# thethomasboyer/PhenDiff

Measured on AMD Instinct MI355X. Metric: img2img images/sec (50-step DDIM invert+denoise, 256x256), higher is better.
Workload: dtype bf16; 1 GPU; configs[2]: 256x256 pipeline_conditional_ddim invert->class-swap->denoise, 50+50 DDIM steps, super_small UNet (random init, seed 0), 3k_steps_clipping_rescaling, 32 images/GPU/step sharded over 1 GPU(s), no collectives; batch_per_gpu=32, global_batch=32, inference_steps=50, image_size=256, hipgraph=True, concurrent_trajectories=1

## Files before the change

### phendiff_amd/csrc/conv_igemm.hip

```cpp
#include <type_traits>
#include <utility>
#include <stdio.h>
#include <stdlib.h>
#include "pd_common.h"
#include "pd_stage.h"
#include "pd_conv.h"

namespace pd {

constexpr int CONV_AR8 = 6;
constexpr int CONV_PRO_DEFAULT = 1;
constexpr int CONV_PRO_WPS = 3;
constexpr int CONV_PRO_START = 8;
template <int... I, typename F> __device__ __forceinline__ void pd_static_for_impl(std::integer_sequence<int, I...>, F&& f) { (f(std::integral_constant<int, I>{}), ...); }
template <int N, typename F> __device__ __forceinline__ void pd_static_for(F&& f) { pd_static_for_impl(std::make_integer_sequence<int, N>{}, f); }
constexpr int PRO_OPS = 37;
constexpr int pro_op_cost(int k) {
  if (k >= 36) return 100;
  const int stg = (k % 18) >> 1;
  return (stg == 3 || stg == 4 || stg == 6 || stg == 7) ? 87 : (stg == 0 ? 60 : (stg == 8 ? 106 : 58));
}
constexpr int pro_ops_done(int S, int NS, int PS0, int NIT) {
  if (S < PS0) return 0;
  if (S >= NS - 1) return NIT * PRO_OPS;
  long long tot = 0;
  for (int k = 0; k < PRO_OPS; ++k) tot += pro_op_cost(k);
  tot *= NIT;
  const long long target = (long long)(S - PS0 + 1) * tot / (NS - PS0);
  int done = 0;
  long long dc = 0;
  while (done < NIT * PRO_OPS && dc + pro_op_cost(done % PRO_OPS) <= target) { dc += pro_op_cost(done % PRO_OPS); ++done; }
  return done;
}
__device__ __forceinline__ unsigned pd_lin_block() { return blockIdx.x + gridDim.x * (blockIdx.y + gridDim.y * blockIdx.z); }
template <typename T, int KS, int STRIDE, int TH, int TW, bool DB, bool TAIL, int NCO = 1, bool PLAIN = false, int PRO = 0, bool STACK = false>
__global__ __launch_bounds__(256, NCO == 2 ? 2 : (PRO ? CONV_PRO_WPS : (((KS == 1 || (KS == 3 && STRIDE == 1 && TH * TW == 256)) && sizeof(T) == 2) ? 3 : 2))) void conv_kernel(const ConvP p) {
  static_assert(PRO == 0 || (!PLAIN && DB && KS == 3 && STRIDE == 1 && sizeof(T) == 2), "compile-time prologue: 16-bit 3x3 stride-1 double-buffered launches");
  static_assert(!TAIL || (DB && KS == 3 && STRIDE == 1), "fused shortcut tail: 3x3 stride-1 double-buffered variant only");
  static_assert(NCO == 1 || (NCO == 2 && DB && KS == 3 && STRIDE == 1), "two output tiles per workgroup: 3x3 stride-1 double-buffered variant only");
  static_assert(!STACK || (KS == 3 && STRIDE == 1 && TW == 8 && TH == 16 && NCO == 1 && !PLAIN && PRO == 0), "stacked 8 x 8 images: the 16 x 8 tile");
  constexpr int SG = STACK ? TH / 8 : 1;
  using E = Elem<T>;
  using Frag = typename E::Frag;
  using SR = typename Stage<T>::R;
  constexpr int TP = TH * TW;
  constexpr int NF = TP / 64;
  constexpr int RPF = 32 / TW;
  constexpr int IN_TH = STACK ? SG * 10 : (TH - 1) * STRIDE + KS;
  constexpr int IN_TW = (TW - 1) * STRIDE + KS;
  constexpr int NPIX = IN_TH * IN_TW;
  constexpr bool M16 = PLAIN && sizeof(T) == 2 && (KS == 3 || KS == 2) && STRIDE == 1 && DB && TW >= 16;
  constexpr int CHB = 32 * E::BYTES;
  constexpr int PITCH = DB ? 2 * CHB + (M16 ? 32 : 16) : CHB + 16;
  constexpr int NIT = (NPIX * 4 + 255) / 256;
  constexpr int TAPS = KS * KS;
  constexpr int KSTEPS = TAPS * 2;
  constexpr int LDS_TILE = DB ? CHB : 0;
  static_assert(RPF >= 1 && TW * RPF == 32, "TW must divide 32");

  extern __shared__ __attribute__((aligned(16))) unsigned char lds[];

  int co_t = blockIdx.y, n = blockIdx.z * SG, bx = blockIdx.x;
  if (!STACK && p.co_major) {
    const int gx = gridDim.x, gxz = gridDim.x * gridDim.z;
    const int idx = xcd_chunk_index((int)pd_lin_block(), gxz * (int)gridDim.y);
    co_t = idx / gxz;
    const int rem = idx - co_t * gxz;
    n = rem / gx; bx = rem - n * gx;
  }
  int tx, ty;
  if (p.tiles_x_shift >= 0) { tx = bx & (p.tiles_x - 1); ty = bx >> p.tiles_x_shift; }
  else { ty = bx / p.tiles_x; tx = bx - ty * p.tiles_x; }
  const int y0 = ty * TH, x0 = tx * TW;

  const int tid = threadIdx.x;
  const int lane = tid & 63;
  const int wave = __builtin_amdgcn_readfirstlane(tid >> 6);
  const int wp = wave >> 1, wc = wave & 1;
  const int r = lane & 31, h = lane >> 5;
  const int ct32 = co_t * (2 * NCO) + wc;
  const bool wave_active = (ct32 * 32) < p.Cout_pad;

  const __amdgpu_buffer_rsrc_t rs0 = __builtin_amdgcn_make_buffer_rsrc((void*)p.x0, 0, p.bytes0, 0x00020000);
  const __amdgpu_buffer_rsrc_t rs1 = __builtin_amdgcn_make_buffer_rsrc((void*)(p.x1 ? p.x1 : p.x0), 0, p.bytes1, 0x00020000);

  const __amdgpu_buffer_rsrc_t rt0 = __builtin_amdgcn_make_buffer_rsrc((void*)(TAIL ? p.t0 : p.x0), 0, TAIL ? p.tbytes0 : p.bytes0, 0x00020000);
  const __amdgpu_buffer_rsrc_t rt1 = __builtin_amdgcn_make_buffer_rsrc((void*)((TAIL && p.t1) ? p.t1 : p.x0), 0, (TAIL && p.t1) ? p.tbytes1 : p.bytes0, 0x00020000);

  const int sub = tid & 3;
  auto stage_pix = [&](int i) { return (tid + 256 * i) >> 2; };
  const int Hc = p.upsample ? p.Hin * 2 : p.Hin;
  const int Wc = p.upsample ? p.Win * 2 : p.Win;
  int spix[NIT];
  constexpr int TAIL_CENTRE = 1 << 30;
  const int ups = p.upsample ? 1 : 0;
  const int ph_mask = p.upsample >= 2 ? 1 : 0, ph_want = p.upsample == 3 ? 1 : 0;
  const int istep = p.in_step, Ws = p.Win * istep;
  const int iy_base = y0 * STRIDE - p.pad, ix_base = x0 * STRIDE - p.pad_x, n_base = n * p.Hin * istep + p.in_oy;
#pragma unroll
  for (int i = 0; i < NIT; ++i) {
    const int pix = stage_pix(i);
    const int u = pix / IN_TW, vv = pix - u * IN_TW;
    const int sj = STACK ? u / 10 : 0, su = u - sj * 10;
    const int iy = STACK ? su - 1 : iy_base + u, ix = ix_base + vv;
    const bool ok = (pix < NPIX) & ((unsigned)iy < (unsigned)Hc) & ((unsigned)ix < (unsigned)Wc) & (!STACK || n + sj < p.B)
                    & (((iy & ph_mask) == (ph_want & ph_mask)) & ((ix & ph_mask) == (ph_want & ph_mask)));
    int v = STACK ? ((n + sj) * 8 + iy) * 8 + ix : (n_base + (iy >> ups) * istep) * Ws + (ix >> ups) * istep + p.in_ox;
    if (TAIL) v |= (((unsigned)((STACK ? su : u) - KS / 2) < (unsigned)(STACK ? 8 : TH)) & ((unsigned)(vv - KS / 2) < (unsigned)TW)) ? TAIL_CENTRE : 0;
    spix[i] = ok ? v : -1;
  }
  const bool affine = PRO || (!PLAIN && p.scale != nullptr);
  const bool do_silu = PRO || (!PLAIN && p.silu != 0);
  const int cin = p.C0 + p.C1;

  SR stage[NIT];
  float sc[8], sh[8];
  bool stage_plain = false;
  auto issue_loads = [&](int chunk) {
    int src, cch;
    if (!TAIL || chunk < p.n_main) { cch = chunk * 32; src = cch < p.C0 ? 0 : 1; if (src == 1) cch -= p.C0; }
    else { cch = (chunk - p.n_main) * 32; src = cch < p.Ct0 ? 2 : 3; if (src == 3) cch -= p.Ct0; }
    stage_plain = TAIL && src >= 2;
    const unsigned cs = src == 0 ? p.C0 : (src == 1 ? p.C1 : (src == 2 ? p.Ct0 : p.Ct1));
    const unsigned cbytes = (unsigned)(cch + sub * 8) * E::BYTES;
#pragma unroll
    for (int i = 0; i < NIT; ++i) {
      const bool want = TAIL ? (stage_plain ? spix[i] >= TAIL_CENTRE : spix[i] >= 0) : spix[i] >= 0;
      const unsigned off = want ? (unsigned)(TAIL ? spix[i] & (TAIL_CENTRE - 1) : spix[i]) * cs * E::BYTES + cbytes : OOB_OFF;
      stage[i] = src == 0 ? Stage<T>::load(rs0, off) : (src == 1 ? Stage<T>::load(rs1, off)
                 : (src == 2 ? Stage<T>::load(rt0, off) : Stage<T>::load(rt1, off)));
    }
    if ((PRO && !stage_plain) || (!PRO && affine && !stage_plain)) {
      const int cg = chunk * 32 + sub * 8;
      const float* ps = p.scale + (size_t)n * cin + cg;
      const float* pb = p.shift + (size_t)n * cin + cg;
      const f32x4 a0 = *(const f32x4*)ps, a1 = *((const f32x4*)ps + 1);
      const f32x4 b0 = *(const f32x4*)pb, b1 = *((const f32x4*)pb + 1);
#pragma unroll
      for (int j = 0; j < 4; ++j) { sc[j] = a0[j]; sc[4 + j] = a1[j]; sh[j] = b0[j]; sh[4 + j] = b1[j]; }
    }
  };
  auto write_piece = [&](int i, unsigned char* buf, bool tail_piece = false) {
    const int pix = stage_pix(i);
    if constexpr (PRO) {
      if (TAIL && tail_piece) {
        if (pix < NPIX && spix[i] >= 0) *(u32x4*)(buf + pix * PITCH + sub * 8 * E::BYTES) = Stage<T>::raw(stage[i]);
        return;
      }
      const u32x4 o = Stage<T>::xform_gs(stage[i], sc, sh);
      const bool ok = pix < NPIX && spix[i] >= 0;
      *(u32x4*)(ok ? buf + pix * PITCH + sub * 8 * E::BYTES : lds + NPIX * PITCH) = o;
    } else
    if (pix < NPIX && spix[i] >= 0)
      Stage<T>::template xform_store<false>(buf + pix * PITCH + sub * 8 * E::BYTES, stage[i], sc, sh, affine && !stage_plain,
                                            do_silu && !stage_plain, true);
  };
  auto zero_padding = [&]() {
#pragma unroll
    for (int i = 0; i < NIT; ++i) {
      const int pix = stage_pix(i);
      if (pix < NPIX && spix[i] < 0) {
        unsigned char* d = lds + pix * PITCH + sub * 8 * E::BYTES;
#pragma unroll
        for (int q = 0; q < (DB ? 2 : 1); ++q)
#pragma unroll
          for (int b16 = 0; b16 < 8 * E::BYTES; b16 += 16) *(u32x4*)(d + q * LDS_TILE + b16) = (u32x4)(0u);
      }
    }
  };

  auto stage_im2col = [&](unsigned char* buf) {
    if constexpr (KS == 1 && STRIDE == 1) {
      const int py = tid / TW, px = tid % TW;
      const int oy = y0 + py, ox = x0 + px;
      const float* src = (const float*)p.x0;
      float v[32];
#pragma unroll
      for (int k = 0; k < 32; ++k) v[k] = 0.f;
#pragma unroll
      for (int ci = 0; ci < 3; ++ci) {
#pragma unroll
        for (int ky = 0; ky < 3; ++ky) {
#pragma unroll
          for (int kx = 0; kx < 3; ++kx) {
            const int iy = oy + ky - 1, ix = ox + kx - 1;
            const bool ok = ci < p.C0r && iy >= 0 && iy < p.Hin && ix >= 0 && ix < p.Win;
            const int cic = min(ci, p.C0r - 1), iyc = min(max(iy, 0), p.Hin - 1), ixc = min(max(ix, 0), p.Win - 1);
            const float xv = src[(((size_t)n * p.C0r + cic) * p.Hin + iyc) * p.Win + ixc];
            v[ci * 9 + ky * 3 + kx] = ok ? xv : 0.f;
          }
        }
      }
#pragma unroll
      for (int q = 0; q < 4; ++q) {
// ... 2 lines not shown
        for (int j = 0; j < 8; ++j) o[j] = v[q * 8 + j];
        E::store(buf + tid * PITCH + q * 8 * E::BYTES, E::pack(o));
      }
    }
  };

  auto frag_row = [&](int fi, int q) { return fi * RPF + q; };
  const int li = lane & 15, lg = lane >> 4;
  constexpr int TJ_STEP = (TW >= 32 ? 16 : IN_TW) * PITCH;
  int rbase[NF];
#pragma unroll
  for (int f = 0; f < NF; ++f) {
    const int fi = wp * NF + f;
    if constexpr (M16) {
      rbase[f] = f == 0 ? ((wp * NF * RPF) * IN_TW + li) * PITCH + lg * 8 * E::BYTES : 0;
    } else {
      const int py = frag_row(fi, r / TW), px = r % TW;
      const int ly = STACK ? py + 2 * (py >> 3) : py * STRIDE;
      rbase[f] = (ly * IN_TW + px * STRIDE) * PITCH + h * 8 * E::BYTES;
    }
  }

  f32x16 acc[NCO][NF];
  f32x4 acq[NCO][NF][4];
  const int main_ksteps = (TAIL ? p.n_main : p.nchunks) * KSTEPS;
  const int all_ksteps = main_ksteps + (TAIL ? p.n_tail * 2 : 0);
  const unsigned wfrag = 512u * E::BYTES;
  const __amdgpu_buffer_rsrc_t rw = __builtin_amdgcn_make_buffer_rsrc((void*)p.w, 0, (unsigned)(p.Cout_pad / 32) * (unsigned)all_ksteps * wfrag, 0x00020000);
  const unsigned wlane = (unsigned)lane * 8u * E::BYTES;
  const unsigned wtile = (unsigned)ct32 * (unsigned)all_ksteps * wfrag;
  const unsigned wstep = 2u * (unsigned)all_ksteps * wfrag;
  auto load_w = [&](int c, int kstep) { return E::load_buf(rw, wlane, wtile + (unsigned)c * wstep + (unsigned)kstep * wfrag); };

  constexpr int AR = (KS == 3 && TW == 8 && STRIDE == 1 && sizeof(T) == 2 && TP <= 128) ? CONV_AR8 : ((KSTEPS % 3 == 0) ? 3 : 2);
  static_assert(KSTEPS % AR == 0, "the ring index is static");
  constexpr int AD = AR - 1;
  Frag aring[AR][NCO];
  static_assert(!M16 || NF % 2 == 0, "M16 walks a fragment pair per half-step");
  Frag aq[2][NCO][2];
  const unsigned wlane16 = (unsigned)(((lg >> 1) * 64 + (lg & 1) * 32 + li) * 16);
  auto load_w16 = [&](int c, int tap_index, int ti) {
    return E::load_buf(rw, wlane16 + (unsigned)ti * 256u, wtile + (unsigned)c * wstep + (unsigned)(2 * tap_index) * wfrag);
  };

  auto mma_chunk = [&](int chunk, const unsigned char* buf, unsigned char* nbuf, auto have_next_c, auto active_c) {
    constexpr int NEXT = (int)decltype(have_next_c)::value;
    constexpr bool HAVE_NEXT = NEXT != 0, NEXT_PLAIN = NEXT == 2;
    constexpr bool ACTIVE = decltype(active_c)::value;
    const int g0 = chunk * KSTEPS;
    Frag bc[NF];
    int piece = 0;
    if constexpr (!PRO) __builtin_amdgcn_iglp_opt(0);
    if constexpr (PRO && ACTIVE) {
      constexpr int NM = NCO * NF;
      constexpr int NS = KSTEPS * NM;
      constexpr int PS0 = CONV_PRO_START < NS - 8 ? CONV_PRO_START : 0;
      f32x2 py[4], pw[4];
      u32x4 po;
      auto piece_op = [&](auto ic, auto kc) __attribute__((always_inline)) {
        constexpr int i = decltype(ic)::value, k = decltype(kc)::value;
        if constexpr (k < 36) {
          constexpr int half = k / 18, kk = k % 18, stg = kk >> 1, j = half * 2 + (kk & 1);
          if constexpr (stg == 0) { const uint32_t wj = Stage<T>::word(stage[i], j); float lo, hi; Pack16<T>::unpack(wj, lo, hi); pw[j].x = lo; pw[j].y = hi; }
          else if constexpr (stg == 1) py[j] = pw[j] * (f32x2){sc[2 * j], sc[2 * j + 1]} + (f32x2){sh[2 * j], sh[2 * j + 1]};
          else if constexpr (stg == 2) pw[j] = py[j] * (f32x2)(-1.4426950408889634f);
          else if constexpr (stg == 3) pw[j].x = __builtin_amdgcn_exp2f(pw[j].x);
          else if constexpr (stg == 4) pw[j].y = __builtin_amdgcn_exp2f(pw[j].y);
          else if constexpr (stg == 5) pw[j] = pw[j] + (f32x2)(1.0f);
          else if constexpr (stg == 6) pw[j].x = __builtin_amdgcn_rcpf(pw[j].x);
          else if constexpr (stg == 7) pw[j].y = __builtin_amdgcn_rcpf(pw[j].y);
          else { const f32x2 o = py[j] * pw[j]; po[j] = Pack16<T>::pack(o.x, o.y); }
          if constexpr (stg == 1) asm volatile("" : "+v"(py[j]));
          else if constexpr (stg == 8) { uint32_t w = po[j]; asm volatile("" : "+v"(w)); po[j] = w; }
          else asm volatile("" : "+v"(pw[j]));
        } else {
          const int pix = stage_pix(i);
          const bool ok = pix < NPIX && spix[i] >= 0;
          *(u32x4*)(ok ? nbuf + pix * PITCH + sub * 8 * E::BYTES : lds + NPIX * PITCH) = NEXT_PLAIN ? Stage<T>::raw(stage[i]) : po;
        }
      };
      auto run_ops = [&](auto s_c) __attribute__((always_inline)) {
        constexpr int S = decltype(s_c)::value;
        if constexpr (NEXT_PLAIN) {
          constexpr int lo = (S * NIT) / NS, hi = ((S + 1) * NIT) / NS;
          pd_static_for<hi - lo>([&](auto gc) __attribute__((always_inline)) {
            piece_op(std::integral_constant<int, lo + decltype(gc)::value>{}, std::integral_constant<int, 36>{});
          });
        } else if constexpr (HAVE_NEXT) {
          constexpr int lo = S == 0 ? 0 : pro_ops_done(S - 1, NS, PS0, NIT), hi = pro_ops_done(S, NS, PS0, NIT);
          pd_static_for<hi - lo>([&](auto gc) __attribute__((always_inline)) {
            constexpr int g = lo + decltype(gc)::value;
            piece_op(std::integral_constant<int, g / PRO_OPS>{}, std::integral_constant<int, g % PRO_OPS>{});
          });
        }
      };
#pragma unroll
      for (int f = 0; f < NF; ++f) bc[f] = E::load(buf + rbase[f]);
      __builtin_amdgcn_sched_barrier(0);
      pd_static_for<NS>([&](auto sc_) __attribute__((always_inline)) {
        constexpr int S = decltype(sc_)::value, ks = S / NM, m = S % NM, f = m / NCO, c = m % NCO;
        constexpr int tapn = (ks + 1) >> 1, sn = (ks + 1) & 1;
        constexpr int toffn = ((tapn / KS) * IN_TW + (tapn % KS)) * PITCH + sn * 16 * E::BYTES;
        if constexpr (m == 0) {
#pragma unroll
          for (int cc = 0; cc < NCO; ++cc) aring[(ks + AD) % AR][cc] = load_w(cc, g0 + ks + AD);
        }
        acc[c][f] = E::mma(aring[ks % AR][c], bc[f], acc[c][f]);
        if constexpr (c == NCO - 1 && ks + 1 < KSTEPS) bc[f] = E::load(buf + rbase[f] + toffn);
        run_ops(sc_);
        __builtin_amdgcn_sched_barrier(0);
      });
    } else
#pragma unroll
    for (int ks = 0; ks < KSTEPS; ++ks) {
      if constexpr (ACTIVE && M16) {
        const int tap = ks >> 1, s = ks & 1;
        if (s == 0) {
#pragma unroll
          for (int c = 0; c < NCO; ++c)
#pragma unroll
            for (int ti = 0; ti < 2; ++ti) aq[(tap + 1) & 1][c][ti] = load_w16(c, chunk * TAPS + tap + 1, ti);
        }
        constexpr int FH = NF >= 2 ? NF / 2 : 1;
        const int toff = ((tap / KS) * IN_TW + (tap % KS)) * PITCH;
        Frag bq[FH][2];
#pragma unroll
        for (int f = 0; f < FH; ++f)
#pragma unroll
          for (int tj = 0; tj < 2; ++tj) bq[f][tj] = E::load(buf + rbase[0] + (s * FH + f) * (RPF * IN_TW * PITCH) + tj * TJ_STEP + toff);
        __builtin_amdgcn_s_setprio(1);
#pragma unroll
        for (int c = 0; c < NCO; ++c)
#pragma unroll
          for (int f = 0; f < FH; ++f)
#pragma unroll
            for (int ti = 0; ti < 2; ++ti)
#pragma unroll
              for (int tj = 0; tj < 2; ++tj)
                acq[c][s * FH + f][2 * ti + tj] = E::mma_16x16x32(aq[tap & 1][c][ti], bq[f][tj], acq[c][s * FH + f][2 * ti + tj]);
        __builtin_amdgcn_s_setprio(0);
      } else if constexpr (ACTIVE) {
#pragma unroll
        for (int c = 0; c < NCO; ++c) aring[(ks + AD) % AR][c] = load_w(c, g0 + ks + AD);
        {
          const int tap = ks >> 1, s = ks & 1;
          const int toff = ((tap / KS) * IN_TW + (tap % KS)) * PITCH + s * 16 * E::BYTES;
#pragma unroll
          for (int f = 0; f < NF; ++f) bc[f] = E::load(buf + rbase[f] + toff);
        }
        __builtin_amdgcn_s_setprio(1);
#pragma unroll
        for (int c = 0; c < NCO; ++c)
#pragma unroll
          for (int f = 0; f < NF; ++f) acc[c][f] = E::mma(aring[ks % AR][c], bc[f], acc[c][f]);
        __builtin_amdgcn_s_setprio(0);
      }
      if constexpr (DB && HAVE_NEXT) {
        const int due = ((ks + 1) * NIT) / KSTEPS;
#pragma unroll
        for (int i = 0; i < NIT; ++i)
          if (i >= piece && i < due) write_piece(i, nbuf);
        piece = due;
// ... 37 lines not shown
      const int kt = main_ksteps + (chunk - p.n_main) * 2;
      Frag a0[NCO], a1[NCO];
#pragma unroll
      for (int c = 0; c < NCO; ++c) { a0[c] = load_w(c, kt); a1[c] = load_w(c, kt + 1); }
      Frag b0[NF], b1[NF];
#pragma unroll
      for (int f = 0; f < NF; ++f) { b0[f] = E::load(buf + rbase[f] + CENTER); b1[f] = E::load(buf + rbase[f] + CENTER + 16 * E::BYTES); }
      __builtin_amdgcn_s_setprio(1);
#pragma unroll
      for (int c = 0; c < NCO; ++c) {
#pragma unroll
        for (int f = 0; f < NF; ++f) acc[c][f] = E::mma(a0[c], b0[f], acc[c][f]);
#pragma unroll
        for (int f = 0; f < NF; ++f) acc[c][f] = E::mma(a1[c], b1[f], acc[c][f]);
      }
      __builtin_amdgcn_s_setprio(0);
    }
    if constexpr (HAVE_NEXT) {
#pragma unroll
      for (int i = 0; i < NIT; ++i) write_piece(i, nbuf, true);
    }
  };
  using std::true_type; using std::false_type;

  f32x4 bt[NCO][4];
  u32x4 tv[NCO][4];
  if constexpr (M16) {
    if (wave_active) {
      const __amdgpu_buffer_rsrc_t rtemb = __builtin_amdgcn_make_buffer_rsrc((void*)(p.temb ? p.temb : p.bias), 0,
          p.temb ? ((unsigned)n * (unsigned)p.temb_stride + (unsigned)p.Cout) * 4u : 0u, 0x00020000);
#pragma unroll
      for (int c = 0; c < NCO; ++c)
#pragma unroll
        for (int ti = 0; ti < 2; ++ti) {
          const int co = (ct32 + 2 * c) * 32 + 16 * ti + 4 * lg;
          bt[c][ti] = *(const f32x4*)(p.bias + co);
          tv[c][ti] = __builtin_amdgcn_raw_buffer_load_b128(rtemb, (unsigned)(n * p.temb_stride + co) * 4u, 0, 0);
        }
    }
  } else
  if (wave_active) {
    const int nt = STACK ? min(n + wp, p.B - 1) : n;
    const __amdgpu_buffer_rsrc_t rtemb = __builtin_amdgcn_make_buffer_rsrc((void*)(p.temb ? p.temb : p.bias), 0,
        p.temb ? ((unsigned)nt * (unsigned)p.temb_stride + (unsigned)p.Cout) * 4u : 0u, 0x00020000);
#pragma unroll
    for (int c = 0; c < NCO; ++c)
#pragma unroll
      for (int g = 0; g < 4; ++g) {
        const int co = (ct32 + 2 * c) * 32 + 8 * g + 4 * h;
        bt[c][g] = *(const f32x4*)(p.bias + co);
        tv[c][g] = __builtin_amdgcn_raw_buffer_load_b128(rtemb, (unsigned)(nt * p.temb_stride + co) * 4u, 0, 0);
      }
  }
  if (!p.im2col3) issue_loads(0);
  if (wave_active) {
#pragma unroll
    for (int c = 0; c < NCO; ++c)
#pragma unroll
      for (int g = 0; g < (M16 ? 2 : 4); ++g)
#pragma unroll
        for (int i = 0; i < 4; ++i) bt[c][g][i] += __uint_as_float(tv[c][g][i]);
  }
  if constexpr (M16) {
#pragma unroll
    for (int c = 0; c < NCO; ++c)
#pragma unroll
      for (int f = 0; f < NF; ++f)
#pragma unroll
        for (int q = 0; q < 4; ++q) acq[c][f][q] = wave_active ? bt[c][q >> 1] : (f32x4)(0.f);
    if (wave_active) {
#pragma unroll
      for (int c = 0; c < NCO; ++c) { aq[0][c][0] = load_w16(c, 0, 0); aq[0][c][1] = load_w16(c, 0, 1); }
    }
  } else {
#pragma unroll
  for (int c = 0; c < NCO; ++c) {
    f32x16 init = (f32x16)(0.f);
    if (wave_active) {
#pragma unroll
      for (int g = 0; g < 4; ++g)
#pragma unroll
        for (int i = 0; i < 4; ++i) init[4 * g + i] = bt[c][g][i];
    }
#pragma unroll
    for (int f = 0; f < NF; ++f) acc[c][f] = init;
  }
  if (wave_active) {
#pragma unroll
    for (int i = 0; i < AD; ++i)
#pragma unroll
      for (int c = 0; c < NCO; ++c) aring[i][c] = load_w(c, i);
  }
  }
  if (!p.im2col3) zero_padding();
  if (DB) {
    if (p.im2col3) {
      stage_im2col(lds);
    } else {
      write_piece(0, lds);
#pragma unroll
      for (int i = 1; i < NIT; ++i) write_piece(i, lds);
    }
    if (p.nchunks > 1) issue_loads(1);
    __syncthreads();
    int chunk = 0;
    const int main_loop_end = TAIL ? (PRO ? p.n_main - 1 : p.n_main) : p.nchunks - 1;
    for (; chunk < main_loop_end; ++chunk) {
      unsigned char* buf = lds + (chunk & 1) * LDS_TILE;
      unsigned char* nbuf = lds + ((chunk + 1) & 1) * LDS_TILE;
      if constexpr (PRO) mma_chunk(chunk, buf, nbuf, true_type{}, true_type{});
      else if (wave_active) mma_chunk(chunk, buf, nbuf, true_type{}, true_type{});
      else mma_chunk(chunk, buf, nbuf, true_type{}, false_type{});
      if (chunk + 2 < p.nchunks) issue_loads(chunk + 2);
      __syncthreads();
    }
    if constexpr (TAIL && PRO) {
      mma_chunk(chunk, lds + (chunk & 1) * LDS_TILE, lds + ((chunk + 1) & 1) * LDS_TILE, std::integral_constant<int, 2>{}, true_type{});
      if (chunk + 2 < p.nchunks) issue_loads(chunk + 2);
      __syncthreads();
      ++chunk;
    }
    if constexpr (TAIL) {
      for (; chunk + 1 < p.nchunks; ++chunk) {
        unsigned char* buf = lds + (chunk & 1) * LDS_TILE;
        unsigned char* nbuf = lds + ((chunk + 1) & 1) * LDS_TILE;
        if (wave_active) mma_tail(chunk, buf, nbuf, true_type{}, true_type{});
        else mma_tail(chunk, buf, nbuf, true_type{}, false_type{});
        if (chunk + 2 < p.nchunks) issue_loads(chunk + 2);
        __syncthreads();
      }
      if (wave_active) mma_tail(chunk, lds + (chunk & 1) * LDS_TILE, lds, false_type{}, true_type{});
    } else {
      if (wave_active) mma_chunk(chunk, lds + (chunk & 1) * LDS_TILE, lds, false_type{}, true_type{});
    }
    __syncthreads();
  } else {
    for (int chunk = 0; chunk < p.nchunks; ++chunk) {
      if (chunk > 0) __syncthreads();
#pragma unroll
      for (int i = 0; i < NIT; ++i) write_piece(i, lds);
      __syncthreads();
      if (chunk + 1 < p.nchunks) issue_loads(chunk + 1);
      if (wave_active) mma_chunk(chunk, lds, lds, false_type{}, true_type{});
    }
  }

  const int co_w = ct32 * 32;
  if (p.out_mode == PD_OUT_NCHW_F32) {
    if (!wave_active) return;
    if constexpr (M16) {
#pragma unroll
      for (int f = 0; f < NF; ++f)
#pragma unroll
        for (int tj = 0; tj < 2; ++tj) {
          const int fi = wp * NF + f, pp = tj * 16 + li;
          const int oy = y0 + fi * RPF + pp / TW, ox = x0 + pp % TW;
          if (oy >= p.Hout || ox >= p.Wout) continue;
#pragma unroll
          for (int ti = 0; ti < 2; ++ti) {
            const int co = co_w + 16 * ti + 4 * lg;
#pragma unroll
            for (int i = 0; i < 4; ++i)
              if (co + i < p.Cout) ((float*)p.y)[(((size_t)n * p.Cout + co + i) * p.Hout + oy) * p.Wout + ox] = acq[0][f][2 * ti + tj][i];
          }
        }
      return;
    }
#pragma unroll
    for (int f = 0; f < NF; ++f) {
      const int fi = wp * NF + f;
      const int oy = y0 + frag_row(fi, r / TW), ox = x0 + r % TW;
      if (oy >= p.Hout || ox >= p.Wout) continue;
#pragma unroll
      for (int g = 0; g < 4; ++g) {
        const int co = co_w + 8 * g + 4 * h;
#pragma unroll
        for (int i = 0; i < 4; ++i)
          if (co + i < p.Cout) ((float*)p.y)[(((size_t)n * p.Cout + co + i) * p.Hout + oy) * p.Wout + ox] = acc[0][f][4 * g + i];
      }
    }
    return;
  }
  constexpr int EP_PITCH = 64 * E::BYTES + 16;
  constexpr int EPC = 16 / E::BYTES;
  constexpr int PPP = 64 / EPC;
  constexpr int PXI = 256 / PPP;
  constexpr int NEP = TP / PXI;
  static_assert(PXI % TW == 0 || TW % PXI == 0, "epilogue piece map");
  const int piece = tid % PPP, prow = tid / PPP;
  const int py0 = prow / TW, px0 = prow % TW;
  const int os = p.out_step, HF = p.Hout * os, WF = p.Wout * os;
  const unsigned out_bytes = (unsigned)p.B * HF * WF * p.Cout * E::BYTES;
  const __amdgpu_buffer_rsrc_t ry = __builtin_amdgcn_make_buffer_rsrc((void*)p.y, 0, p.out_mode == PD_OUT_NHWC ? out_bytes : 0u, 0x00020000);
  const __amdgpu_buffer_rsrc_t rres = __builtin_amdgcn_make_buffer_rsrc((void*)(p.residual ? p.residual : p.y), 0, p.residual ? out_bytes : 0u, 0x00020000);
  const unsigned px_bytes = (unsigned)p.Cout * E::BYTES * os, row_bytes = (unsigned)WF * p.Cout * E::BYTES * os;
// ... 79 lines not shown
        }
      }
    }
  } else if (co < p.Cout) {
#pragma unroll
    for (int it = 0; it < NEP; ++it) {
      const int plin = it * PXI + prow;
      const int oy = y0 + plin / TW, ox = x0 + plin % TW;
      if (oy >= p.Hout || ox >= p.Wout) continue;
      const u32x4 v = *(const u32x4*)(lds + plin * EP_PITCH + piece * 16);
      const int Cq = p.heads * 8;
      const int which = co / Cq, cc = co - which * Cq;
      const size_t N = (size_t)p.Hout * p.Wout;
      const size_t tok = (size_t)oy * p.Wout + ox;
      *(u32x4*)((T*)p.y + ((((size_t)which * p.B + n) * p.heads + (cc >> 3)) * N + tok) * 8 + (cc & 7)) = v;
    }
  }
  if (p.stats) {
    float* red = (float*)(lds + TP * EP_PITCH);
#pragma unroll
    for (int sg = 0; sg < SG; ++sg) {
      if (sg > 0) __syncthreads();
#pragma unroll
      for (int q = 0; q < 2 * EPC / 4; ++q) {
        f32x4 v4;
#pragma unroll
        for (int j = 0; j < 4; ++j) { const int e = q * 4 + j; v4[j] = e < EPC ? ssum[sg][e] : ssq[sg][e - EPC]; }
        *(f32x4*)(red + tid * (2 * EPC) + q * 4) = v4;
      }
      __syncthreads();
      if (tid < 128) {
        const int c = tid >> 1, which = tid & 1;
        const int pc = c / EPC, j = c % EPC;
        const int cog = co_tile * 64 + c;
        float tot = 0.f;
#pragma unroll 8
        for (int pr = 0; pr < PXI; ++pr) tot += red[(pr * PPP + pc) * (2 * EPC) + which * EPC + j];
        if (cog < p.Cout && n + sg < p.B) {
          const int tile = p.stat_tile_base + ty * p.tiles_x + tx;
          p.stats[(((size_t)(n + sg) * p.stat_tiles + tile) * p.Cout + cog) * 2 + which] = tot;
        }
      }
    }
  }
  }
}

template <typename T, int KS, int STRIDE, int TH, int TW, bool TAIL = false, int NCO = 1, bool PLAIN = false, int PRO = 0, bool STACK = false>
static int launch_conv(const ConvP& p, hipStream_t st) {
  constexpr int IN_TH = STACK ? (TH / 8) * 10 : (TH - 1) * STRIDE + KS, IN_TW = (TW - 1) * STRIDE + KS;
  constexpr int PITCH = 32 * Elem<T>::BYTES + 16;
  constexpr int LDS_TILE = ((IN_TH * IN_TW * PITCH + 15) / 16) * 16;
  constexpr bool DB = 2 * LDS_TILE <= 100 * 1024 && STRIDE != 2;
  constexpr bool M16 = PLAIN && sizeof(T) == 2 && (KS == 3 || KS == 2) && STRIDE == 1 && TW >= 16;
  constexpr int LDS_DB = ((IN_TH * IN_TW * (2 * 32 * Elem<T>::BYTES + (M16 ? 32 : 16)) + 15) / 16) * 16;
  constexpr int EPI_BYTES = TH * TW * (64 * Elem<T>::BYTES + 16) + 256 * 64;
  constexpr int LDS_MAIN = (DB ? LDS_DB : LDS_TILE) + (PRO ? 16 : 0);
  constexpr int LDS_BYTES = LDS_MAIN > EPI_BYTES ? LDS_MAIN : EPI_BYTES;
  static_assert(LDS_BYTES <= 160 * 1024, "tile too large");
  static_assert(NCO == 1 || DB, "NCO = 2 is a double-buffered variant");
  auto kern = conv_kernel<T, KS, STRIDE, TH, TW, DB, TAIL, NCO, PLAIN, PRO, STACK>;
  if (LDS_BYTES > 64 * 1024) {
    static LdsAttr attr;
    if (!ensure_lds(attr, kern, LDS_BYTES)) { set_error("pd_conv: cannot reserve %d bytes of LDS", LDS_BYTES); return PD_ERR_LAUNCH; }
  }
  ConvP q = p;
  q.tiles_x = (p.Wout + TW - 1) / TW;
  q.tiles_y = STACK ? 1 : (p.Hout + TH - 1) / TH;
  q.tiles_x_shift = -1;
  for (int sft = 0; sft < 16; ++sft) if ((1 << sft) == q.tiles_x) q.tiles_x_shift = sft;
  q.n_co_tiles = (p.Cout_pad + 63) / 64;
  if (q.stat_tiles == 0) q.stat_tiles = q.tiles_x * q.tiles_y;
  else { q.stat_tiles *= q.tiles_x * q.tiles_y; q.stat_tile_base *= q.tiles_x * q.tiles_y; }
  {
    const long long es = (long long)sizeof(T), cin = (long long)p.C0 + p.C1;
    const long long wbytes = (long long)p.Cout_pad * cin * KS * KS * es, abytes = (long long)p.B * p.Hin * p.Win * cin * es;
    const long long blocks = (long long)q.tiles_x * q.tiles_y * (q.n_co_tiles / NCO) * p.B;
    const int env = diag_env("PD_CONV_XCD", 0);
    q.co_major = !STACK && blocks >= 64 && blocks < (1ll << 30) && !p.im2col3 && (env == 1 || (env == 2 && wbytes > abytes));
  }
  hipLaunchKernelGGL(kern, dim3(q.tiles_x * q.tiles_y, q.n_co_tiles / NCO, STACK ? (p.B + TH / 8 - 1) / (TH / 8) : p.B), dim3(256), LDS_BYTES, st, q);
  PD_LAUNCH_CHECK();
  return PD_OK;
}

static void tile_shape(int ksize, int stride, int hout, int wout, int* th, int* tw) {
  const int tp = (ksize == 3 && stride == 1 && wout <= 8 && hout <= 8) ? 64
                 : ((ksize == 3 && stride == 2) || (ksize == 3 && stride == 1 && wout < 16 && hout <= 16)) ? 128 : 256;
  *tw = wout >= 32 ? 32 : (wout >= 16 ? 16 : 8);
  *th = tp / *tw;
}

template <typename T>
static int dispatch_conv(const ConvP& p, int ksize, int stride, hipStream_t st) {
  const int w = p.Wout;
  if (ksize == 3 && stride == 1) {
    const bool tiny = p.Hout <= 16;
    if constexpr (sizeof(T) == 2) {
      const int nco_env = diag_env("PD_CONV_NCO", 0);
      static int cus_of[16] = {0};
      int dev = 0;
      if (hipGetDevice(&dev) != hipSuccess || dev < 0 || dev >= 16) dev = 0;
      if (cus_of[dev] == 0) {
        int c = 0;
        if (hipDeviceGetAttribute(&c, hipDeviceAttributeMultiprocessorCount, dev) != hipSuccess || c <= 0) c = 256;
        cus_of[dev] = c;
      }
      const int cus = cus_of[dev];
      bool nco2 = false;
      if (w >= 32 && p.Cout_pad % 128 == 0 && p.Cout == p.Cout_pad && p.out_mode != PD_OUT_NCHW_F32) {
        const long long wgs1 = (long long)((p.Wout + 31) / 32) * ((p.Hout + 7) / 8) * (p.Cout_pad / 64) * p.B, wgs2 = wgs1 / 2;
        auto eff = [](long long wgs, long long slots) { return (double)wgs / (double)(((wgs + slots - 1) / slots) * slots); };
        const double speed2 = (p.scale != nullptr && p.C0 + p.C1 >= 128) ? 1.05 : 0.84;
        nco2 = nco_env ? nco_env == 2 : eff(wgs2, 2ll * cus) * speed2 > eff(wgs1, 3ll * cus);
      }
      const bool plain_off = diag_env("PD_CONV_PLAIN", 1) == 0;
      const bool plain = !plain_off && p.scale == nullptr && !p.silu && !p.im2col3 && w >= 16;
      const int pro_lvl = diag_env("PD_CONV_PRO", CONV_PRO_DEFAULT);
      const bool gs = p.scale != nullptr && p.silu != 0 && !p.im2col3 && w >= 32 && p.Cout_pad % 64 == 0 && p.out_mode != PD_OUT_NCHW_F32;
      if (nco2 && gs && pro_lvl >= 1)
        return p.n_tail > 0 ? launch_conv<T, 3, 1, 8, 32, true, 2, false, 1>(p, st) : launch_conv<T, 3, 1, 8, 32, false, 2, false, 1>(p, st);
      if (nco2) return p.n_tail > 0 ? launch_conv<T, 3, 1, 8, 32, true, 2>(p, st) : launch_conv<T, 3, 1, 8, 32, false, 2>(p, st);
      if (plain) {
        if (p.n_tail > 0) return w >= 32 ? launch_conv<T, 3, 1, 8, 32, true, 1, true>(p, st) : launch_conv<T, 3, 1, 16, 16, true, 1, true>(p, st);
        return w >= 32 ? launch_conv<T, 3, 1, 8, 32, false, 1, true>(p, st) : launch_conv<T, 3, 1, 16, 16, false, 1, true>(p, st);
      }
    }
    const bool one8 = p.Hout <= 8 && w <= 8;
    const bool stack = p.Hout == 8 && w == 8 && p.Hin == 8 && p.Win == 8 && !p.upsample && p.in_step == 1 && p.out_step == 1 && p.pad == 1 && p.pad_x == 1 &&
                       p.scale == nullptr && !p.silu && !p.im2col3 && p.out_mode == PD_OUT_NHWC && p.B >= 2 && diag_env("PD_CONV_STACK", 0) != 0;
    if (stack) return p.n_tail > 0 ? launch_conv<T, 3, 1, 16, 8, true, 1, false, 0, true>(p, st) : launch_conv<T, 3, 1, 16, 8, false, 1, false, 0, true>(p, st);
    if (p.n_tail > 0) {
      if (w >= 32) return launch_conv<T, 3, 1, 8, 32, true>(p, st);
      if (w >= 16) return launch_conv<T, 3, 1, 16, 16, true>(p, st);
      if (one8) return launch_conv<T, 3, 1, 8, 8, true>(p, st);
      if (tiny) return launch_conv<T, 3, 1, 16, 8, true>(p, st);
      return launch_conv<T, 3, 1, 32, 8, true>(p, st);
    }
    if (w >= 32) return launch_conv<T, 3, 1, 8, 32>(p, st);
    if (w >= 16) return launch_conv<T, 3, 1, 16, 16>(p, st);
    if (one8) return launch_conv<T, 3, 1, 8, 8>(p, st);
    if (tiny) return launch_conv<T, 3, 1, 16, 8>(p, st);
    return launch_conv<T, 3, 1, 32, 8>(p, st);
  }
  if (ksize == 3 && stride == 2) {
    if (w >= 32) return launch_conv<T, 3, 2, 4, 32>(p, st);
    if (w >= 16) return launch_conv<T, 3, 2, 8, 16>(p, st);
    return launch_conv<T, 3, 2, 16, 8>(p, st);
  }
  if (ksize == 2 && stride == 1) {
    if (w >= 32) return launch_conv<T, 2, 1, 8, 32, false, 1, true>(p, st);
    if (w >= 16) return launch_conv<T, 2, 1, 16, 16, false, 1, true>(p, st);
    set_error("pd_conv: the 2x2 phase form needs Wout >= 16");
    return PD_ERR_UNSUPPORTED;
  }
  if (ksize == 1 && stride == 1) {
    if (w >= 32) return launch_conv<T, 1, 1, 8, 32>(p, st);
    if (w >= 16) return launch_conv<T, 1, 1, 16, 16>(p, st);
    return launch_conv<T, 1, 1, 32, 8>(p, st);
  }
  set_error("pd_conv: unsupported ksize=%d stride=%d", ksize, stride);
  return PD_ERR_UNSUPPORTED;
}

}

extern "C" int pd_conv(const pd_conv_args* a, void* stream) {
  using namespace pd;
  PD_CHECK(a != nullptr, PD_ERR_ARG, "pd_conv: null args");
  PD_CHECK(a->dtype == PD_F32 || a->dtype == PD_BF16 || a->dtype == PD_F16, PD_ERR_ARG, "pd_conv: bad dtype %d", a->dtype);
  PD_CHECK(a->B > 0 && a->Hin > 0 && a->Win > 0 && a->Hout > 0 && a->Wout > 0, PD_ERR_SHAPE, "pd_conv: bad spatial shape");
  PD_CHECK(a->C0 > 0 && a->C0 % 32 == 0 && a->C1 >= 0 && a->C1 % 32 == 0, PD_ERR_SHAPE,
           "pd_conv: C0=%d C1=%d must be multiples of 32", a->C0, a->C1);
  PD_CHECK(a->Cout > 0 && a->Cout_pad >= a->Cout && a->Cout_pad % 32 == 0, PD_ERR_SHAPE, "pd_conv: bad Cout/Cout_pad");
// ... 83 lines not shown
```

Baseline: 15.70 images/s.

## Use 16x16x32 MFMA form in fused GroupNorm-SiLU prologue conv kernels

Adds a PRO==2 variant of the two-tile 8x32 3x3 conv that runs its main loop on 16x16x32 MFMA fragments, like the plain M16 path, while keeping the fused GroupNorm/SiLU prologue of the next chunk interleaved. Per-sample scale/shift rows are staged once into LDS and read per piece rather than reloaded from global memory each chunk. Pixel indices are spilled to LDS and reloaded near the end to relieve register pressure. The prologue-op spreading weights slots unevenly to match the new MFMA schedule. This raises LDS use and is gated to C<=512 without a shortcut tail.

Result: no change. 15.79 images/s (median of 6 runs) (+0.6%).

```diff
diff --git a/phendiff_amd/csrc/conv_igemm.hip b/phendiff_amd/csrc/conv_igemm.hip
--- a/phendiff_amd/csrc/conv_igemm.hip
+++ b/phendiff_amd/csrc/conv_igemm.hip
@@ -12,6 +12,7 @@
 constexpr int CONV_PRO_DEFAULT = 1;
 constexpr int CONV_PRO_WPS = 3;
 constexpr int CONV_PRO_START = 8;
+constexpr int CONV_PRO_M16_DEFAULT = 1;
 template <int... I, typename F> __device__ __forceinline__ void pd_static_for_impl(std::integer_sequence<int, I...>, F&& f) { (f(std::integral_constant<int, I>{}), ...); }
 template <int N, typename F> __device__ __forceinline__ void pd_static_for(F&& f) { pd_static_for_impl(std::make_integer_sequence<int, N>{}, f); }
 constexpr int PRO_OPS = 37;
@@ -20,13 +21,16 @@
   const int stg = (k % 18) >> 1;
   return (stg == 3 || stg == 4 || stg == 6 || stg == 7) ? 87 : (stg == 0 ? 60 : (stg == 8 ? 106 : 58));
 }
-constexpr int pro_ops_done(int S, int NS, int PS0, int NIT) {
+constexpr int pro_slot_weight(int S, bool M16Q) { return !M16Q ? 1 : (S % 32 < 4 ? 0 : (S % 4 == 3 ? 1 : 2)); }
+constexpr int pro_ops_done(int S, int NS, int PS0, int NIT, bool M16Q = false) {
   if (S < PS0) return 0;
   if (S >= NS - 1) return NIT * PRO_OPS;
   long long tot = 0;
   for (int k = 0; k < PRO_OPS; ++k) tot += pro_op_cost(k);
   tot *= NIT;
-  const long long target = (long long)(S - PS0 + 1) * tot / (NS - PS0);
+  long long wdone = 0, wall = 0;
+  for (int s = PS0; s < NS; ++s) { wall += pro_slot_weight(s, M16Q); if (s <= S) wdone += pro_slot_weight(s, M16Q); }
+  const long long target = wdone * tot / wall;
   int done = 0;
   long long dc = 0;
   while (done < NIT * PRO_OPS && dc + pro_op_cost(done % PRO_OPS) <= target) { dc += pro_op_cost(done % PRO_OPS); ++done; }
@@ -36,6 +40,7 @@
 template <typename T, int KS, int STRIDE, int TH, int TW, bool DB, bool TAIL, int NCO = 1, bool PLAIN = false, int PRO = 0, bool STACK = false>
 __global__ __launch_bounds__(256, NCO == 2 ? 2 : (PRO ? CONV_PRO_WPS : (((KS == 1 || (KS == 3 && STRIDE == 1 && TH * TW == 256)) && sizeof(T) == 2) ? 3 : 2))) void conv_kernel(const ConvP p) {
   static_assert(PRO == 0 || (!PLAIN && DB && KS == 3 && STRIDE == 1 && sizeof(T) == 2), "compile-time prologue: 16-bit 3x3 stride-1 double-buffered launches");
+  static_assert(PRO != 2 || (NCO == 2 && TH == 8 && TW == 32), "16x16x32 form of the prologue: the two-tile 8 x 32 launches");
   static_assert(!TAIL || (DB && KS == 3 && STRIDE == 1), "fused shortcut tail: 3x3 stride-1 double-buffered variant only");
   static_assert(NCO == 1 || (NCO == 2 && DB && KS == 3 && STRIDE == 1), "two output tiles per workgroup: 3x3 stride-1 double-buffered variant only");
   static_assert(!STACK || (KS == 3 && STRIDE == 1 && TW == 8 && TH == 16 && NCO == 1 && !PLAIN && PRO == 0), "stacked 8 x 8 images: the 16 x 8 tile");
@@ -49,7 +54,7 @@
   constexpr int IN_TH = STACK ? SG * 10 : (TH - 1) * STRIDE + KS;
   constexpr int IN_TW = (TW - 1) * STRIDE + KS;
   constexpr int NPIX = IN_TH * IN_TW;
-  constexpr bool M16 = PLAIN && sizeof(T) == 2 && (KS == 3 || KS == 2) && STRIDE == 1 && DB && TW >= 16;
+  constexpr bool M16 = (PLAIN || PRO == 2) && sizeof(T) == 2 && (KS == 3 || KS == 2) && STRIDE == 1 && DB && TW >= 16;
   constexpr int CHB = 32 * E::BYTES;
   constexpr int PITCH = DB ? 2 * CHB + (M16 ? 32 : 16) : CHB + 16;
   constexpr int NIT = (NPIX * 4 + 255) / 256;
@@ -109,6 +114,21 @@
     if (TAIL) v |= (((unsigned)((STACK ? su : u) - KS / 2) < (unsigned)(STACK ? 8 : TH)) & ((unsigned)(vv - KS / 2) < (unsigned)TW)) ? TAIL_CENTRE : 0;
     spix[i] = ok ? v : -1;
   }
+  constexpr int AFF_ROW = 512, AFF_OFF = NPIX * PITCH + 16, SPIX_OFF = AFF_OFF + 2 * AFF_ROW * 4;
+  unsigned ok_mask = 0;
+  if constexpr (PRO) {
+#pragma unroll
+    for (int i = 0; i < NIT; ++i) {
+      *(int*)(lds + SPIX_OFF + (i * 256 + tid) * 4) = spix[i];
+      ok_mask |= (stage_pix(i) < NPIX && spix[i] >= 0) ? 1u << i : 0u;
+    }
+  }
+  auto reload_spix = [&](auto ic) __attribute__((always_inline)) {
+    constexpr int i = decltype(ic)::value;
+    int a = SPIX_OFF + tid * 4;
+    asm volatile("" : "+v"(a));
+    spix[i] = *(const int*)(lds + a + i * 1024);
+  };
   const bool affine = PRO || (!PLAIN && p.scale != nullptr);
   const bool do_silu = PRO || (!PLAIN && p.silu != 0);
   const int cin = p.C0 + p.C1;
@@ -116,7 +136,7 @@
   SR stage[NIT];
   float sc[8], sh[8];
   bool stage_plain = false;
-  auto issue_loads = [&](int chunk) {
+  auto issue_loads = [&](int chunk, auto first_c) {
     int src, cch;
     if (!TAIL || chunk < p.n_main) { cch = chunk * 32; src = cch < p.C0 ? 0 : 1; if (src == 1) cch -= p.C0; }
     else { cch = (chunk - p.n_main) * 32; src = cch < p.Ct0 ? 2 : 3; if (src == 3) cch -= p.Ct0; }
@@ -130,7 +150,7 @@
       stage[i] = src == 0 ? Stage<T>::load(rs0, off) : (src == 1 ? Stage<T>::load(rs1, off)
                  : (src == 2 ? Stage<T>::load(rt0, off) : Stage<T>::load(rt1, off)));
     }
-    if ((PRO && !stage_plain) || (!PRO && affine && !stage_plain)) {
+    if ((PRO && decltype(first_c)::value) || (!PRO && affine && !stage_plain)) {
       const int cg = chunk * 32 + sub * 8;
       const float* ps = p.scale + (size_t)n * cin + cg;
       const float* pb = p.shift + (size_t)n * cin + cg;
@@ -140,6 +160,12 @@
       for (int j = 0; j < 4; ++j) { sc[j] = a0[j]; sc[4 + j] = a1[j]; sh[j] = b0[j]; sh[4 + j] = b1[j]; }
     }
   };
+  u32x4 aff_v = (u32x4)(0u);
+  auto load_affine_rows = [&]() {
+    const __amdgpu_buffer_rsrc_t ra = __builtin_amdgcn_make_buffer_rsrc((void*)((wp ? p.shift : p.scale) + (size_t)n * cin), 0, (unsigned)cin * 4u, 0x00020000);
+    aff_v = __builtin_amdgcn_raw_buffer_load_b128(ra, (unsigned)(tid & 127) * 16u, 0, 0);
+  };
+  auto store_affine_rows = [&]() { *(u32x4*)(lds + AFF_OFF + wp * (AFF_ROW * 4) + (tid & 127) * 16) = aff_v; };
   auto write_piece = [&](int i, unsigned char* buf, bool tail_piece = false) {
     const int pix = stage_pix(i);
     if constexpr (PRO) {
@@ -248,17 +274,28 @@
     int piece = 0;
     if constexpr (!PRO) __builtin_amdgcn_iglp_opt(0);
     if constexpr (PRO && ACTIVE) {
-      constexpr int NM = NCO * NF;
+      constexpr int NM = NCO * NF * (M16 ? 2 : 1);
       constexpr int NS = KSTEPS * NM;
       constexpr int PS0 = CONV_PRO_START < NS - 8 ? CONV_PRO_START : 0;
+      constexpr int FH = NF >= 2 ? NF / 2 : 1;
+      constexpr int FRAG_STEP = RPF * IN_TW * PITCH;
+      Frag bq[FH][2];
       f32x2 py[4], pw[4];
       u32x4 po;
+      f32x4 tsc, tsh;
+      int aff_a = AFF_OFF + ((chunk + 1) * 32 + sub * 8) * 4;
+      auto read_affine = [&](auto hc) __attribute__((always_inline)) {
+        constexpr int H = decltype(hc)::value;
+        asm volatile("" : "+v"(aff_a));
+        tsc = *(const f32x4*)(lds + aff_a + (H & 1) * 16);
+        tsh = *(const f32x4*)(lds + aff_a + (H & 1) * 16 + AFF_ROW * 4);
+      };
       auto piece_op = [&](auto ic, auto kc) __attribute__((always_inline)) {
         constexpr int i = decltype(ic)::value, k = decltype(kc)::value;
         if constexpr (k < 36) {
           constexpr int half = k / 18, kk = k % 18, stg = kk >> 1, j = half * 2 + (kk & 1);
           if constexpr (stg == 0) { const uint32_t wj = Stage<T>::word(stage[i], j); float lo, hi; Pack16<T>::unpack(wj, lo, hi); pw[j].x = lo; pw[j].y = hi; }
-          else if constexpr (stg == 1) py[j] = pw[j] * (f32x2){sc[2 * j], sc[2 * j + 1]} + (f32x2){sh[2 * j], sh[2 * j + 1]};
+          else if constexpr (stg == 1) py[j] = pw[j] * (f32x2){tsc[2 * (kk & 1)], tsc[2 * (kk & 1) + 1]} + (f32x2){tsh[2 * (kk & 1)], tsh[2 * (kk & 1) + 1]};
           else if constexpr (stg == 2) pw[j] = py[j] * (f32x2)(-1.4426950408889634f);
           else if constexpr (stg == 3) pw[j].x = __builtin_amdgcn_exp2f(pw[j].x);
           else if constexpr (stg == 4) pw[j].y = __builtin_amdgcn_exp2f(pw[j].y);
@@ -269,9 +306,10 @@
           if constexpr (stg == 1) asm volatile("" : "+v"(py[j]));
           else if constexpr (stg == 8) { uint32_t w = po[j]; asm volatile("" : "+v"(w)); po[j] = w; }
           else asm volatile("" : "+v"(pw[j]));
+          if constexpr (kk == 4 && 2 * i + half + 1 < 2 * NIT) read_affine(std::integral_constant<int, 2 * i + half + 1>{});
         } else {
           const int pix = stage_pix(i);
-          const bool ok = pix < NPIX && spix[i] >= 0;
+          const bool ok = (ok_mask >> i) & 1u;
           *(u32x4*)(ok ? nbuf + pix * PITCH + sub * 8 * E::BYTES : lds + NPIX * PITCH) = NEXT_PLAIN ? Stage<T>::raw(stage[i]) : po;
         }
       };
@@ -283,27 +321,45 @@
             piece_op(std::integral_constant<int, lo + decltype(gc)::value>{}, std::integral_constant<int, 36>{});
           });
         } else if constexpr (HAVE_NEXT) {
-          constexpr int lo = S == 0 ? 0 : pro_ops_done(S - 1, NS, PS0, NIT), hi = pro_ops_done(S, NS, PS0, NIT);
+          constexpr int lo = S == 0 ? 0 : pro_ops_done(S - 1, NS, PS0, NIT, M16), hi = pro_ops_done(S, NS, PS0, NIT, M16);
           pd_static_for<hi - lo>([&](auto gc) __attribute__((always_inline)) {
             constexpr int g = lo + decltype(gc)::value;
             piece_op(std::integral_constant<int, g / PRO_OPS>{}, std::integral_constant<int, g % PRO_OPS>{});
           });
         }
       };
-#pragma unroll
-      for (int f = 0; f < NF; ++f) bc[f] = E::load(buf + rbase[f]);
+      if constexpr (M16) {
+#pragma unroll
+        for (int f = 0; f < FH; ++f)
+#pragma unroll
+          for (int tj = 0; tj < 2; ++tj) bq[f][tj] = E::load(buf + rbase[0] + f * FRAG_STEP + tj * TJ_STEP);
+      } else {
+#pragma unroll
+        for (int f = 0; f < NF; ++f) bc[f] = E::load(buf + rbase[f]);
+      }
+      if constexpr (HAVE_NEXT && !NEXT_PLAIN) read_affine(std::integral_constant<int, 0>{});
       __builtin_amdgcn_sched_barrier(0);
       pd_static_for<NS>([&](auto sc_) __attribute__((always_inline)) {
-        constexpr int S = decltype(sc_)::value, ks = S / NM, m = S % NM, f = m / NCO, c = m % NCO;
+        constexpr int S = decltype(sc_)::value, ks = S / NM, m = S % NM;
         constexpr int tapn = (ks + 1) >> 1, sn = (ks + 1) & 1;
-        constexpr int toffn = ((tapn / KS) * IN_TW + (tapn % KS)) * PITCH + sn * 16 * E::BYTES;
-        if constexpr (m == 0) {
-#pragma unroll
-          for (int cc = 0; cc < NCO; ++cc) aring[(ks + AD) % AR][cc] = load_w(cc, g0 + ks + AD);
-        }
-        acc[c][f] = E::mma(aring[ks % AR][c], bc[f], acc[c][f]);
-        if constexpr (c == NCO - 1 && ks + 1 < KSTEPS) bc[f] = E::load(buf + rbase[f] + toffn);
+        if constexpr (M16) {
+          constexpr int tap = ks >> 1, s = ks & 1, b = m / (2 * NCO), f = b / 2, tj = b % 2, c = (m % (2 * NCO)) / 2, ti = m % 2;
+          constexpr int toffn = ((tapn / KS) * IN_TW + (tapn % KS)) * PITCH;
+          if constexpr (s == 0 && m < 2 * NCO) aq[(tap + 1) & 1][m / 2][m % 2] = load_w16(m / 2, chunk * TAPS + tap + 1, m % 2);
+          acq[c][s * FH + f][2 * ti + tj] = E::mma_16x16x32(aq[tap & 1][c][ti], bq[f][tj], acq[c][s * FH + f][2 * ti + tj]);
+          if constexpr (m % (2 * NCO) == 2 * NCO - 1 && ks + 1 < KSTEPS) bq[f][tj] = E::load(buf + rbase[0] + (sn * FH + f) * FRAG_STEP + tj * TJ_STEP + toffn);
+        } else {
+          constexpr int f = m / NCO, c = m % NCO;
+          constexpr int toffn = ((tapn / KS) * IN_TW + (tapn % KS)) * PITCH + sn * 16 * E::BYTES;
+          if constexpr (m == 0) {
+#pragma unroll
+            for (int cc = 0; cc < NCO; ++cc) aring[(ks + AD) % AR][cc] = load_w(cc, g0 + ks + AD);
+          }
+          acc[c][f] = E::mma(aring[ks % AR][c], bc[f], acc[c][f]);
+          if constexpr (c == NCO - 1 && ks + 1 < KSTEPS) bc[f] = E::load(buf + rbase[f] + toffn);
+        }
         run_ops(sc_);
+        if constexpr (HAVE_NEXT && S >= NS - 8 && S - (NS - 8) < NIT) reload_spix(std::integral_constant<int, S - (NS - 8)>{});
         __builtin_amdgcn_sched_barrier(0);
       });
     } else
@@ -447,7 +503,8 @@
         tv[c][g] = __builtin_amdgcn_raw_buffer_load_b128(rtemb, (unsigned)(nt * p.temb_stride + co) * 4u, 0, 0);
       }
   }
-  if (!p.im2col3) issue_loads(0);
+  if constexpr (PRO) load_affine_rows();
+  if (!p.im2col3) issue_loads(0, std::true_type{});
   if (wave_active) {
 #pragma unroll
     for (int c = 0; c < NCO; ++c)
@@ -488,6 +545,7 @@
   }
   }
   if (!p.im2col3) zero_padding();
+  if constexpr (PRO) store_affine_rows();
   if (DB) {
     if (p.im2col3) {
       stage_im2col(lds);
@@ -496,7 +554,7 @@
 #pragma unroll
       for (int i = 1; i < NIT; ++i) write_piece(i, lds);
     }
-    if (p.nchunks > 1) issue_loads(1);
+    if (p.nchunks > 1) issue_loads(1, std::false_type{});
     __syncthreads();
     int chunk = 0;
     const int main_loop_end = TAIL ? (PRO ? p.n_main - 1 : p.n_main) : p.nchunks - 1;
@@ -506,12 +564,12 @@
       if constexpr (PRO) mma_chunk(chunk, buf, nbuf, true_type{}, true_type{});
       else if (wave_active) mma_chunk(chunk, buf, nbuf, true_type{}, true_type{});
       else mma_chunk(chunk, buf, nbuf, true_type{}, false_type{});
-      if (chunk + 2 < p.nchunks) issue_loads(chunk + 2);
+      if (chunk + 2 < p.nchunks) issue_loads(chunk + 2, std::false_type{});
       __syncthreads();
     }
     if constexpr (TAIL && PRO) {
       mma_chunk(chunk, lds + (chunk & 1) * LDS_TILE, lds + ((chunk + 1) & 1) * LDS_TILE, std::integral_constant<int, 2>{}, true_type{});
-      if (chunk + 2 < p.nchunks) issue_loads(chunk + 2);
+      if (chunk + 2 < p.nchunks) issue_loads(chunk + 2, std::false_type{});
       __syncthreads();
       ++chunk;
     }
@@ -521,7 +579,7 @@
         unsigned char* nbuf = lds + ((chunk + 1) & 1) * LDS_TILE;
         if (wave_active) mma_tail(chunk, buf, nbuf, true_type{}, true_type{});
         else mma_tail(chunk, buf, nbuf, true_type{}, false_type{});
-        if (chunk + 2 < p.nchunks) issue_loads(chunk + 2);
+        if (chunk + 2 < p.nchunks) issue_loads(chunk + 2, std::false_type{});
         __syncthreads();
       }
       if (wave_active) mma_tail(chunk, lds + (chunk & 1) * LDS_TILE, lds, false_type{}, true_type{});
@@ -535,7 +593,7 @@
 #pragma unroll
       for (int i = 0; i < NIT; ++i) write_piece(i, lds);
       __syncthreads();
-      if (chunk + 1 < p.nchunks) issue_loads(chunk + 1);
+      if (chunk + 1 < p.nchunks) issue_loads(chunk + 1, std::false_type{});
       if (wave_active) mma_chunk(chunk, lds, lds, false_type{}, true_type{});
     }
   }
@@ -721,10 +779,10 @@
   constexpr int PITCH = 32 * Elem<T>::BYTES + 16;
   constexpr int LDS_TILE = ((IN_TH * IN_TW * PITCH + 15) / 16) * 16;
   constexpr bool DB = 2 * LDS_TILE <= 100 * 1024 && STRIDE != 2;
-  constexpr bool M16 = PLAIN && sizeof(T) == 2 && (KS == 3 || KS == 2) && STRIDE == 1 && TW >= 16;
+  constexpr bool M16 = (PLAIN || PRO == 2) && sizeof(T) == 2 && (KS == 3 || KS == 2) && STRIDE == 1 && TW >= 16;
   constexpr int LDS_DB = ((IN_TH * IN_TW * (2 * 32 * Elem<T>::BYTES + (M16 ? 32 : 16)) + 15) / 16) * 16;
   constexpr int EPI_BYTES = TH * TW * (64 * Elem<T>::BYTES + 16) + 256 * 64;
-  constexpr int LDS_MAIN = (DB ? LDS_DB : LDS_TILE) + (PRO ? 16 : 0);
+  constexpr int LDS_MAIN = (DB ? LDS_DB : LDS_TILE) + (PRO ? 16 + 2 * 512 * 4 + ((IN_TH * IN_TW * 4 + 255) / 256) * 1024 : 0);
   constexpr int LDS_BYTES = LDS_MAIN > EPI_BYTES ? LDS_MAIN : EPI_BYTES;
   static_assert(LDS_BYTES <= 160 * 1024, "tile too large");
   static_assert(NCO == 1 || DB, "NCO = 2 is a double-buffered variant");
@@ -786,9 +844,11 @@
       const bool plain_off = diag_env("PD_CONV_PLAIN", 1) == 0;
       const bool plain = !plain_off && p.scale == nullptr && !p.silu && !p.im2col3 && w >= 16;
       const int pro_lvl = diag_env("PD_CONV_PRO", CONV_PRO_DEFAULT);
-      const bool gs = p.scale != nullptr && p.silu != 0 && !p.im2col3 && w >= 32 && p.Cout_pad % 64 == 0 && p.out_mode != PD_OUT_NCHW_F32;
-      if (nco2 && gs && pro_lvl >= 1)
+      const bool gs = p.scale != nullptr && p.silu != 0 && !p.im2col3 && w >= 32 && p.Cout_pad % 64 == 0 && p.out_mode != PD_OUT_NCHW_F32 && p.C0 + p.C1 <= 512;
+      if (nco2 && gs && pro_lvl >= 1) {
+        if (p.n_tail == 0 && diag_env("PD_CONV_PRO_M16", CONV_PRO_M16_DEFAULT) != 0) return launch_conv<T, 3, 1, 8, 32, false, 2, false, 2>(p, st);
         return p.n_tail > 0 ? launch_conv<T, 3, 1, 8, 32, true, 2, false, 1>(p, st) : launch_conv<T, 3, 1, 8, 32, false, 2, false, 1>(p, st);
+      }
       if (nco2) return p.n_tail > 0 ? launch_conv<T, 3, 1, 8, 32, true, 2>(p, st) : launch_conv<T, 3, 1, 8, 32, false, 2>(p, st);
       if (plain) {
         if (p.n_tail > 0) return w >= 32 ? launch_conv<T, 3, 1, 8, 32, true, 1, true>(p, st) : launch_conv<T, 3, 1, 16, 16, true, 1, true>(p, st);
```
